# msaelices/mojo-regex

Measured on AMD Instinct MI355X. Metric: GB/s input scanned + matches/sec, 1M x 1KiB batch, [a-z]+\d+ DFA, higher is better.
Workload: dtype u8

## Files before the change

mojo_regex_amd/csrc/mrx_kernels.hip:

```cpp
#include <hip/hip_runtime.h>
#include <atomic>
#include <map>
#include <type_traits>
#include <unordered_map>
#include <chrono>

#include <cstdio>
#include <cstdlib>
#include <cstring>
#include <mutex>
#include <string>
#include <vector>

#include "../../include/mrx.h"
#include "../../include/mrx_testing.h"
#include "mrx_device.hpp"
#include "mrx_host_batch.hpp"
#include "mrx_internal.hpp"
#include "mrx_lookback.hpp"
#include "mrx_rec12.hpp"
#include "mrx_decode_bits.hpp"

using namespace mrx;

// ... 2186 lines not shown
      if (t < 0) len = 0;
      if (len > 0) addr = (uintptr_t)(data + o0);
      const int m0 = len > 0 ? (int)(addr & (CH - 1)) : 0;
      const uintptr_t rb = (addr & ~(uintptr_t)(CH - 1)) - (uintptr_t)shift;
      len_o = len; mis_o = shift + m0; flen_o = shift + m0 + len;
      *(uint4*)(tile + lane * kRowPitch + CH) =
          make_uint4((uint32_t)rb, (uint32_t)((uint64_t)rb >> 32), len > 0 ? (uint32_t)flen_o : 0u, (uint32_t)shift);
    };
    constexpr int KJ = kDynTexts / 64;
    int64_t offr[KJ + 1];
    int lenr[KJ];
#pragma unroll
    for (int j = 0; j <= KJ; ++j) {
      const int64_t t = T0 + 64 * j + lane < T1 ? T0 + 64 * j + lane : T1;
      offr[j] = vlen ? offsets[t < T1 ? t : T1 - 1] : offsets[t];
      if (j < KJ) lenr[j] = vlen ? vlen[t < T1 ? t : T1 - 1] : 0;
    }
    auto off_of = [&](int ti) -> int64_t {
      int64_t v = __shfl(offr[0], ti & 63);
#pragma unroll
      for (int j = 1; j <= KJ; ++j) { const int64_t u = __shfl(offr[j], ti & 63); v = (ti >> 6) == j ? u : v; }
      return v;
    };
    if (!vlen) {
#pragma unroll
      for (int j = 0; j < KJ; ++j) {
        const int64_t up = __shfl_down(offr[j], 1), wrap = __shfl(offr[j + 1], 0);
        lenr[j] = (int)((lane == 63 ? wrap : up) - offr[j]);
      }
    }
    auto len_of = [&](int ti) -> int {
      int v = __shfl(lenr[0], ti & 63);
#pragma unroll
      for (int j = 1; j < KJ; ++j) { const int u = __shfl(lenr[j], ti & 63); v = (ti >> 6) == j ? u : v; }
      return v;
    };
    uint16_t* perm = perm_all[wave];
    int* hist = hist_all[wave];
    {
      int mylen[KJ], tmax = 0;
#pragma unroll
      for (int j = 0; j < KJ; ++j) {
        const int ti = 64 * j + lane;
        const int l = len_of(ti < ntask ? ti : 0);
        mylen[j] = ti < ntask ? l : 0;
        tmax = max(tmax, mylen[j]);
      }
      for (int off = 32; off > 0; off >>= 1) tmax = max(tmax, __shfl_xor(tmax, off));
      const int sh = tmax >= 32 ? 32 - __builtin_clz((unsigned)tmax) - 5 : 0;
      __builtin_amdgcn_wave_barrier();
      if (lane < 32) hist[lane] = 0;
      __builtin_amdgcn_fence(__ATOMIC_RELEASE, "wavefront");
      __builtin_amdgcn_wave_barrier();
      __builtin_amdgcn_fence(__ATOMIC_ACQUIRE, "wavefront");
      int slot[KJ], cls[KJ];
#pragma unroll
      for (int j = 0; j < KJ; ++j) {
        cls[j] = 31 - (mylen[j] >> sh);
        slot[j] = 64 * j + lane < ntask ? atomicAdd(&hist[cls[j]], 1) : 0;
      }
      __builtin_amdgcn_fence(__ATOMIC_RELEASE, "wavefront");
      __builtin_amdgcn_wave_barrier();
      __builtin_amdgcn_fence(__ATOMIC_ACQUIRE, "wavefront");
      int hv = lane < 32 ? hist[lane] : 0, incl = hv;
#pragma unroll
      for (int d = 1; d < 32; d <<= 1) { const int v = __shfl_up(incl, d); if (lane >= d) incl += v; }
      __builtin_amdgcn_wave_barrier();
      if (lane < 32) hist[lane] = incl - hv;
      __builtin_amdgcn_fence(__ATOMIC_RELEASE, "wavefront");
      __builtin_amdgcn_wave_barrier();
      __builtin_amdgcn_fence(__ATOMIC_ACQUIRE, "wavefront");
#pragma unroll
      for (int j = 0; j < KJ; ++j)
        if (64 * j + lane < ntask) perm[hist[cls[j]] + slot[j]] = (uint16_t)(64 * j + lane);
      __builtin_amdgcn_fence(__ATOMIC_RELEASE, "wavefront");
      __builtin_amdgcn_wave_barrier();
      __builtin_amdgcn_fence(__ATOMIC_ACQUIRE, "wavefront");
    }
    {
      const int ti = active ? (int)perm[lane] : 0;
      const int64_t o0 = off_of(ti);
      const int l0 = len_of(ti);
      my_text = T0 + ti;
      describe(active ? my_text : -1, o0, l0, 0, my_len, mis, flen);
    }
    __builtin_amdgcn_fence(__ATOMIC_RELEASE, "wavefront");
    __builtin_amdgcn_wave_barrier();
    __builtin_amdgcn_fence(__ATOMIC_ACQUIRE, "wavefront");
    uint32_t q4 = 0;
    int start = 0, cnt = 0, wtotal = 0;
    int wrec = 0;
    bool done = false;
    int res_s = -1, res_e = -1;
    EvRec* wave_recs = MODE == ST_RECORDS ? recs + rec_region_dyn(offsets[T0], task) : nullptr;
    uint4 v[NL];
#define MRX_DYN_LOAD(CB)                                                                  \
    do {                                                                                  \
      _Pragma("unroll") for (int j_ = 0; j_ < NL; ++j_) {                                  \
        const uint4 rs_ = *(const uint4*)(tile + (RPI * j_ + rsub) * kRowPitch + CH);      \
        uint32_t fo_ = (uint32_t)(CB) + seg * 16;                                          \
        if (fo_ >= rs_.z) fo_ = rs_.w;       \
        v[j_] = MRX_LDG((const uint4*)((const uint8_t*)(((uint64_t)rs_.y << 32) | rs_.x) + fo_)); \
      }                                                                                    \
    } while (0)
    MRX_DYN_LOAD(0);
    uint8_t* wr = tile + rsub * kRowPitch + seg * 16;
    for (int cbase = 0;; cbase += CH) {
#pragma unroll
      for (int j = 0; j < NL; ++j) *(uint4*)(wr + j * RPI * kRowPitch) = v[j];
      __builtin_amdgcn_fence(__ATOMIC_RELEASE, "wavefront");
      __builtin_amdgcn_wave_barrier();
      __builtin_amdgcn_fence(__ATOMIC_ACQUIRE, "wavefront");
      const bool fin = active && (flen <= cbase + CH || (MODE == ST_SEARCH && done));
      const uint64_t fm = __ballot(fin);
      int64_t n_text = -1;
      int n_len = 0, n_mis = 0, n_flen = 0;
      if (fm) {
        const int rank = __builtin_amdgcn_mbcnt_hi((uint32_t)(fm >> 32), __builtin_amdgcn_mbcnt_lo((uint32_t)fm, 0));
        const int cpos = next + rank;
        const int cti = cpos < ntask ? (int)perm[cpos] : 0;
        const int64_t c0 = off_of(cti);
        const int cl = len_of(cti);
        if (fin) {
          n_text = cpos < ntask ? T0 + cti : -1;
          describe(n_text, c0, cl, cbase + CH, n_len, n_mis, n_flen);
        }
        next += __builtin_popcountll(fm);
        __builtin_amdgcn_fence(__ATOMIC_RELEASE, "wavefront");
        __builtin_amdgcn_wave_barrier();
        __builtin_amdgcn_fence(__ATOMIC_ACQUIRE, "wavefront");
      }
      const bool any_next = __any((active && !fin) || n_text >= 0);
      if (any_next) MRX_DYN_LOAD(cbase + CH);

      const int lim = active ? flen - cbase : 0;
      const int lo = active ? mis - cbase : 0;
      const bool all_inside = __all(lim >= CH && lo <= 0);
      uint32_t F_even = 0, meta_even = 0, sp_even = 0;
      constexpr int kUnroll = MODE == ST_COUNT ? 2 : CH / 16;
#pragma unroll kUnroll
      for (int g = 0; g < CH / 16; ++g) {
        const uint4 wv = *(const uint4*)(tile + lane * kRowPitch + g * 16);
        uint32_t words[4] = {wv.x, wv.y, wv.z, wv.w};
        if (!all_inside) {
          const int a = min(max(lo - g * 16, 0), 16), b = min(max(lim - g * 16, 0), 16);
          const uint4 pa = pmask[a], pb = pmask[b > a ? b : a];
          const uint32_t m[4] = {pb.x & ~pa.x, pb.y & ~pa.y, pb.z & ~pa.z, pb.w & ~pa.w};
#pragma unroll
          for (int j = 0; j < 4; ++j) words[j] = (words[j] & m[j]) | (fillw & ~m[j]);
        }
        uint32_t F = 0;
        if (AUTO == 4) {
          uint32_t cc[16], pi[8];
#pragma unroll
          for (int k = 0; k < 16; ++k) cc[k] = cls_lds[(words[k >> 2] >> ((k & 3) * 8)) & 0xFFu];
#pragma unroll
          for (int k = 0; k < 8; ++k) pi[k] = (cc[2 * k] << p.st_cshift) | cc[2 * k + 1];
#pragma unroll
          for (int k = 0; k < 8; ++k) {
            const uint32_t e = pair_lds[q4 + pi[k]];
            q4 = e >> 4;
            F = __builtin_amdgcn_alignbit(e, F, 4);
          }
        } else if (AUTO == 2) {
          uint32_t cc[16];
#pragma unroll
          for (int k = 0; k < 16; ++k) cc[k] = cls_lds[(words[k >> 2] >> ((k & 3) * 8)) & 0xFFu];
#pragma unroll
          for (int k = 0; k < 16; ++k) {
            const uint32_t e = tr_lds[q4 + cc[k]];
            q4 = e >> 2;
            F = __builtin_amdgcn_alignbit(e, F, 2);
          }
        } else if (AUTO == 3) {
#pragma unroll
          for (int h = 0; h < 2; ++h) {
            uint64_t cw[8];
#pragma unroll
            for (int k = 0; k < 8; ++k) cw[k] = col64_lds[(words[(8 * h + k) >> 2] >> ((k & 3) * 8)) & 0xFFu];
#pragma unroll
            for (int k = 0; k < 8; ++k) {
              const uint32_t e = (uint32_t)(cw[k] >> q4);
              q4 = e & 0x38u;
              F = __builtin_amdgcn_alignbit(e, F, 2);
            }
          }
        } else {
          uint32_t cv[16];
#pragma unroll
          for (int k = 0; k < 16; ++k) cv[k] = col_lds[(words[k >> 2] >> ((k & 3) * 8)) & 0xFFu];
#pragma unroll
          for (int k = 0; k < 16; ++k) {
            const uint32_t e = cv[k] >> q4;
            q4 = e & 0xCu;
            F = __builtin_amdgcn_alignbit(e, F, 2);
          }
        }
        const uint32_t em = F & 0xAAAAAAAAu;
        const uint32_t ns = F & 0x55555555u;
        const int gbase = cbase + g * 16 - mis;
        const uint32_t tix = (uint32_t)(my_text - T0) << kDynShift;
        if (MODE == ST_RECORDS && REC32) {
          if ((g & 1) == 0) {
            F_even = F;
            sp_even = (uint32_t)start | ((uint32_t)(gbase + kRecPosBias) << 16);
            meta_even = tix | ((uint32_t)cnt & kDynBeforeMask);
          } else {
            const bool any = ((F_even | F) & 0xAAAAAAAAu) != 0u;
            const uint64_t has = __ballot(any);
            if (has) {
              if (any) {
                const int rank = __builtin_amdgcn_mbcnt_hi((uint32_t)(has >> 32), __builtin_amdgcn_mbcnt_lo((uint32_t)has, 0));
                *(uint4*)(wave_recs + wrec + rank) = make_uint4(F_even, F, sp_even, meta_even);
              }
              wrec += __builtin_popcountll(has);
            }
          }
        } else if (MODE == ST_RECORDS) {
          const uint64_t has = __ballot(em != 0);
          if (has) {
            if (em) {
              const int rank = __builtin_amdgcn_mbcnt_hi((uint32_t)(has >> 32), __builtin_amdgcn_mbcnt_lo((uint32_t)has, 0));
              *(uint4*)(wave_recs + wrec + rank) = make_uint4(F, (uint32_t)start, (uint32_t)gbase, tix | ((uint32_t)cnt & kDynBeforeMask));
            }
            wrec += __builtin_popcountll(has);
          }
        }
        if (MODE == ST_SEARCH) {
          if (!done && em) {
            const int kk = __builtin_ctz(em) >> 1;
            const uint32_t nsb = ns & ((1u << (2 * kk)) - 1u);
            res_s = nsb ? gbase + ((31 - __builtin_clz(nsb)) >> 1) : start;
            res_e = gbase + kk;
            if (p.st_fixed_len > 0) res_s = res_e - p.st_fixed_len;
            done = true;
          }
        }
        cnt += __builtin_popcount(em);
        if (ns) start = gbase + ((31 - __builtin_clz(ns)) >> 1);
      }
      __builtin_amdgcn_wave_barrier();
      {
        const bool tail = fin && accepting(q4) && !(MODE == ST_SEARCH && done);
        if (MODE == ST_RECORDS) {
          const uint64_t has = __ballot(tail);
          if (has) {
            if (tail) {
              const int rank = __builtin_amdgcn_mbcnt_hi((uint32_t)(has >> 32), __builtin_amdgcn_mbcnt_lo((uint32_t)has, 0));
              const uint32_t meta = ((uint32_t)(my_text - T0) << kDynShift) | ((uint32_t)cnt & kDynBeforeMask);
              if (REC32) *(uint4*)(wave_recs + wrec + rank) = make_uint4(2u, 0u, (uint32_t)start | ((uint32_t)(my_len + kRecPosBias) << 16), meta);
              else *(uint4*)(wave_recs + wrec + rank) = make_uint4(2u, (uint32_t)start, (uint32_t)my_len, meta);
            }
            wrec += __builtin_popcountll(has);
          }
        }
        if (fin) {
          if (tail) ++cnt;
          if (MODE == ST_SEARCH) {
            if (!done && tail) { res_s = p.st_fixed_len > 0 ? my_len - p.st_fixed_len : start; res_e = my_len; }
            out_s[my_text] = res_s;
            out_e[my_text] = res_e;
          } else {
            counts[my_text] = cnt;
            wtotal += cnt;
          }
          my_text = n_text; active = n_text >= 0;
          my_len = n_len; mis = n_mis; flen = active ? n_flen : 0;
          q4 = 0; start = 0; cnt = 0; done = false; res_s = -1; res_e = -1;
        }
      }
      if (!any_next) break;
    }
#undef MRX_DYN_LOAD
    if (MODE == ST_RECORDS) {
      for (int off = 32; off > 0; off >>= 1) wtotal += __shfl_xor(wtotal, off);
      if (lane == 0) { wave_nrecs[task] = wrec; wave_nrecs[ntasks + task] = wtotal; }
    }
  }
}

__global__ __launch_bounds__(kBlock) void k_fused_init(unsigned long long* __restrict__ ctrl, int64_t words,
                                                       FusedArgs* __restrict__ dst, FusedArgs args) {
  for (int64_t i = (int64_t)blockIdx.x * blockDim.x + threadIdx.x; i < words; i += (int64_t)gridDim.x * blockDim.x)
    ctrl[i] = 0ull;
  if (blockIdx.x == 0 && threadIdx.x == 0) *dst = args;
}

#ifndef MRX_DECODE_TILE
#define MRX_DECODE_TILE 2048
#endif
constexpr int kDecodeTile = MRX_DECODE_TILE;
#ifndef MRX_DECODE_BATCH
#define MRX_DECODE_BATCH 8
#endif
constexpr int kDecodeBatch = MRX_DECODE_BATCH;

constexpr int kScanBlock = 256;
constexpr int kScanItems = 8;
constexpr int kScanTile = kScanBlock * kScanItems;

#ifndef MRX_DYN_DECODE_TILE
#define MRX_DYN_DECODE_TILE 2048
#endif
template <bool PACK16, bool VBASE = false, bool REC32 = false, bool DYN = false, int TILE = kDecodeTile, bool REC12 = false,
          bool LEAN = false>
__global__ __launch_bounds__(kBlock) void k_decode(int64_t n, const int32_t* __restrict__ wave_nrecs,
                                                   const EvRec* __restrict__ recs, int64_t rec_row,
                                                   const int64_t* __restrict__ offsets,
                                                   const int32_t* __restrict__ counts,
                                                   const int64_t* __restrict__ wave_base,
                                                   const int64_t* __restrict__ scan_block_sums,
                                                   int64_t* __restrict__ prefix,
                                                   int32_t* __restrict__ spans, int64_t span_cap,
                                                   int fixed_len, int64_t* __restrict__ total_out,
                                                   const int32_t* __restrict__ vbase = nullptr,
                                                   const int64_t* __restrict__ base = nullptr, int reverse = 0) {
  static_assert(!(PACK16 && VBASE), "text-relative positions of a long text do not fit 16 bits");
  static_assert(!(DYN && VBASE), "pieces are not handed out dynamically");
  static_assert(!REC12 || (REC32 && PACK16 && !VBASE && !DYN), "12-byte records: short texts at a fixed aligned pitch");
  static_assert(!LEAN || (REC32 && PACK16 && !VBASE && !DYN), "lean pass: two-word records, 16-bit positions, static tasks");
  using Slot = typename std::conditional<PACK16, uint32_t, int2>::type;
  __shared__ Slot tile_all[kBlock / 64][TILE];
  __shared__ int dense_upto[kBlock / 64][64];
  constexpr int kDecodeTile = TILE, kDecodeDirect = 3 * TILE;
  __shared__ int rel_all[DYN ? kBlock / 64 : 1][DYN ? kDynTexts : 1];
  constexpr int kTexts = DYN ? kDynTexts : 64;
  constexpr uint32_t kBefore = DYN ? kDynBeforeMask : kRecBeforeMask;
  constexpr int kTextShift = DYN ? kDynShift : 26;
  const int lane = threadIdx.x & 63;
  Slot* tile = tile_all[threadIdx.x >> 6];
  int* rel_lds = rel_all[DYN ? (threadIdx.x >> 6) : 0];
  const int64_t nw = (n + kTexts - 1) / kTexts;
  const int waves_per_block = blockDim.x >> 6;
  for (int64_t w0 = (int64_t)blockIdx.x * waves_per_block + (threadIdx.x >> 6); w0 < nw;
       w0 += (int64_t)gridDim.x * waves_per_block) {
    const int64_t w = reverse ? nw - 1 - w0 : w0;
    const int64_t first = w * kTexts;
    const int64_t i = first + lane;
    int64_t pre0 = wave_base[w] + (base ? *base : 0);
    {
      const int64_t tiles_before = w / kScanTile;
      int64_t part = 0;
      for (int64_t b = lane; b < tiles_before; b += 64) part += scan_block_sums[b];
      for (int off = 32; off > 0; off >>= 1) part += __shfl_xor(part, off);
      pre0 += part;
    }
    int my_rel = 0, total_spans = 0;
    if (DYN) {
      __builtin_amdgcn_wave_barrier();
      int carry = 0;
      for (int sb = 0; sb < kDynTexts; sb += 64) {
        const int64_t t = first + sb + lane;
        const int c = t < n ? counts[t] : 0;
        int incl = c;
#pragma unroll
        for (int d = 1; d < 64; d <<= 1) {
          const int v = __shfl_up(incl, d);
          if (lane >= d) incl += v;
        }
        rel_lds[sb + lane] = carry + incl - c;
        if (t < n) prefix[t] = pre0 + carry + incl - c;
        if (t == n - 1) { prefix[n] = pre0 + carry + incl; *total_out = pre0 + carry + incl; }
        carry += __shfl(incl, 63);
      }
      total_spans = carry;
      __builtin_amdgcn_fence(__ATOMIC_RELEASE, "wavefront");
      __builtin_amdgcn_wave_barrier();
      __builtin_amdgcn_fence(__ATOMIC_ACQUIRE, "wavefront");
    } else {
    const int my_cnt = i < n ? counts[i] : 0;
    int incl = my_cnt;
#pragma unroll
    for (int d = 1; d < 64; d <<= 1) {
      const int v = __shfl_up(incl, d);
      if (lane >= d) incl += v;
    }
    my_rel = incl - my_cnt;
    total_spans = __shfl(incl, 63);
    if (i < n) prefix[i] = pre0 + my_rel;
    if (i == n - 1) { prefix[n] = pre0 + incl; *total_out = pre0 + incl; }
    }
    const int total_recs = wave_nrecs[w];
    const EvRec* wave_recs = recs + (DYN ? rec_region_dyn(offsets[first], w)
                                         : offsets ? rec_region_start(offsets[first], w) : first * rec_row);
    const uint32_t* wave_recs12 = REC12 ? (const uint32_t*)recs + 3 * (first * rec_row) : nullptr;
    const int my_vb = (VBASE && i < n) ? vbase[i] : 0;
    if (total_spans > kDecodeDirect) {
      constexpr int kRowCap = (DYN || !PACK16) ? 0 : kDecodeTile / 64;
      int done_t = 0;
      for (int j = 0; j < total_recs; j += 64 * kDecodeBatch) {
        EvRec rr[kDecodeBatch];
#pragma unroll
        for (int u = 0; u < kDecodeBatch; ++u) {
          const int o = j + u * 64 + lane;
          rr[u].F = 0; rr[u].start = 0; rr[u].pos_base = 0; rr[u].meta = 0;
          if (o < total_recs) {
            if (REC12) {
              const uint32_t* q_ = wave_recs12 + 3 * o;
              rr[u].F = mrx_ldg32(q_); rr[u].start = (int32_t)mrx_ldg32(q_ + 1); rr[u].meta = mrx_ldg32(q_ + 2);
            } else {
            const uint4 q_ = mrx_ldg((const uint4*)(wave_recs + o));
            rr[u].F = q_.x; rr[u].start = (int32_t)q_.y; rr[u].pos_base = (int32_t)q_.z; rr[u].meta = q_.w;
            }
          }
        }
        if (kRowCap > 0) {
          dense_upto[threadIdx.x >> 6][lane] = done_t;
          __builtin_amdgcn_fence(__ATOMIC_RELEASE, "wavefront");
          __builtin_amdgcn_wave_barrier();
          __builtin_amdgcn_fence(__ATOMIC_ACQUIRE, "wavefront");
        }
#pragma unroll
        for (int u = 0; u < kDecodeBatch; ++u) {
          EvRec r = rr[u];
          const int txt = DYN ? 0 : (int)(r.meta >> 26);
          const int rel_t = DYN ? rel_lds[r.meta >> kTextShift] : __shfl(my_rel, txt);
          if (VBASE) { const int vb = __shfl(my_vb, (int)(r.meta >> 26)); r.start += vb; r.pos_base += vb; }
          const int done_r = kRowCap > 0 ? __shfl(done_t, txt) : 0;
          int within = REC12 ? rec12_before(r.meta) : (int)(r.meta & kBefore);
          int64_t dst = pre0 + rel_t + within;
          uint32_t Fw = r.F;
          int pb = REC12 ? 32 * rec12_pair(r.meta) : REC32 ? (int)((uint32_t)r.pos_base >> 16) - kRecPosBias : r.pos_base;
          int rstart = REC12 ? rec12_start(r.meta) : REC32 ? (int)((uint32_t)r.pos_base & 0xFFFFu) : r.start;
#pragma unroll
          for (int half = 0; half < (REC32 ? 2 : 1); ++half) {
            uint32_t em = Fw & 0xAAAAAAAAu;
            const uint32_t ns = Fw & 0x55555555u;
            while (em) {
              const int kk = __builtin_ctz(em) >> 1;
              const uint32_t nsb = ns & ((1u << (2 * kk)) - 1u);
              int st = nsb ? pb + ((31 - __builtin_clz(nsb)) >> 1) : rstart;
              if (fixed_len > 0) st = pb + kk - fixed_len;
              const int slot = within - done_r;
              if (kRowCap > 0 && slot < kRowCap) {
                if constexpr (PACK16) tile[txt * (kRowCap > 0 ? kRowCap : 1) + slot] = ((uint32_t)st << 16) | (uint32_t)(pb + kk);
              } else if (dst < span_cap) {
                *(int2*)(spans + 2 * dst) = make_int2(st, pb + kk);
              }
              ++dst; ++within;
              em &= em - 1;
            }
            if (REC32) {
              if (ns) rstart = pb + ((31 - __builtin_clz(ns)) >> 1);
              pb += 16;
              Fw = (uint32_t)r.start;
            }
          }
          if (kRowCap > 0 && (r.F | (REC32 ? (uint32_t)r.start : 0u)) != 0u) atomicMax(&dense_upto[threadIdx.x >> 6][txt], within);
        }
        if constexpr (PACK16 && !DYN) {
          __builtin_amdgcn_fence(__ATOMIC_RELEASE, "wavefront");
          __builtin_amdgcn_wave_barrier();
          __builtin_amdgcn_fence(__ATOMIC_ACQUIRE, "wavefront");
          const int upto_t = dense_upto[threadIdx.x >> 6][lane];
          const int64_t row_dst = pre0 + my_rel + done_t;
          int row_n = upto_t - done_t;
          if (row_n > kRowCap) row_n = kRowCap;
          for (int r_ = 0; r_ < 64; ++r_) {
            const int n_r = __shfl(row_n, r_);
            if (n_r <= 0) continue;
            const int64_t d_r = __shfl(row_dst, r_);
            if (lane < n_r && d_r + lane < span_cap) {
              const uint32_t v = (uint32_t)tile[r_ * (kRowCap > 0 ? kRowCap : 1) + lane];
              mrx_stg_span(spans + 2 * (d_r + lane), (int)(v >> 16), (int)(v & 0xFFFFu));
            }
          }
          done_t = upto_t;
          __builtin_amdgcn_wave_barrier();
        }
      }
      continue;
    }
    if constexpr (LEAN) {
      if (total_spans <= kDecodeTile) {
        const int nrec = __builtin_amdgcn_readfirstlane(total_recs), nspan = __builtin_amdgcn_readfirstlane(total_spans);
        const int last_rec = nrec - 1;
        auto lean_pass = [&](auto fixed_tag) {
          constexpr bool FIXED = decltype(fixed_tag)::value;
          for (int j = 0; j < nrec; j += 64 * kDecodeBatch) {
            uint32_t fe[kDecodeBatch], fo[kDecodeBatch], m2[kDecodeBatch], m3[kDecodeBatch];
#pragma unroll
            for (int u = 0; u < kDecodeBatch; ++u) {
              const int o = j + u * 64 + lane;
              const int oc = o < last_rec ? o : last_rec;
              if (REC12) {
                const uint32_t* q_ = wave_recs12 + 3 * oc;
                fe[u] = mrx_ldg32(q_); fo[u] = mrx_ldg32(q_ + 1); m3[u] = mrx_ldg32(q_ + 2); m2[u] = 0;
              } else {
                const uint4 q_ = mrx_ldg((const uint4*)(wave_recs + oc));
                fe[u] = q_.x; fo[u] = q_.y; m2[u] = q_.z; m3[u] = q_.w;
              }
            }
#pragma unroll
            for (int u = 0; u < kDecodeBatch; ++u) {
              if (j + u * 64 >= nrec) break;
              const bool mine = j + u * 64 + lane < nrec;
              const uint32_t f_even = mine ? fe[u] : 0u, f_odd = mine ? fo[u] : 0u;
              const uint32_t meta = m3[u];
              const int rel_t = __shfl(my_rel, (int)(meta >> 26));
              uint32_t* tp = tile + (rel_t + (REC12 ? rec12_before(meta) : (int)(meta & kBefore)));
              const int pb = REC12 ? 32 * rec12_pair(meta) : (int)(m2[u] >> 16) - kRecPosBias;
              const int rstart = REC12 ? rec12_start(meta) : (int)(m2[u] & 0xFFFFu);
              auto emit = [&](int st, int end) { *tp++ = ((uint32_t)st << 16) | (uint32_t)end; };
              decode_expand_record<FIXED>(f_even, f_odd, rstart, pb, fixed_len, emit);
            }
          }
        };
        if (fixed_len > 0) lean_pass(std::true_type{}); else lean_pass(std::false_type{});
        __builtin_amdgcn_fence(__ATOMIC_RELEASE, "wavefront");
        __builtin_amdgcn_wave_barrier();
        __builtin_amdgcn_fence(__ATOMIC_ACQUIRE, "wavefront");
        for (int k = lane; k < nspan; k += 64) {
          const int64_t dst = pre0 + k;
          if (dst < span_cap) { const uint32_t v = tile[k]; mrx_stg_span(spans + 2 * dst, (int)(v >> 16), (int)(v & 0xFFFFu)); }
        }
        __builtin_amdgcn_wave_barrier();
        continue;
      }
    }
    for (int tb = 0; tb < total_spans; tb += kDecodeTile) {
      for (int j = 0; j < total_recs; j += 64 * kDecodeBatch) {
        EvRec rr[kDecodeBatch];
#pragma unroll
        for (int u = 0; u < kDecodeBatch; ++u) {
          const int o = j + u * 64 + lane;
          rr[u].F = 0; rr[u].start = 0; rr[u].pos_base = 0; rr[u].meta = 0;
          if (o < total_recs) {
            if (REC12) {
              const uint32_t* q_ = wave_recs12 + 3 * o;
              rr[u].F = mrx_ldg32(q_); rr[u].start = (int32_t)mrx_ldg32(q_ + 1); rr[u].meta = mrx_ldg32(q_ + 2);
            } else {
            const uint4 q_ = mrx_ldg((const uint4*)(wave_recs + o));
            rr[u].F = q_.x; rr[u].start = (int32_t)q_.y; rr[u].pos_base = (int32_t)q_.z; rr[u].meta = q_.w;
            }
          }
        }
#pragma unroll
        for (int u = 0; u < kDecodeBatch; ++u) {
          EvRec r = rr[u];
          const int rel_t = DYN ? rel_lds[r.meta >> kTextShift] : __shfl(my_rel, (int)(r.meta >> 26));
          if (VBASE) { const int vb = __shfl(my_vb, (int)(r.meta >> 26)); r.start += vb; r.pos_base += vb; }
          int dst = rel_t + (REC12 ? rec12_before(r.meta) : (int)(r.meta & kBefore)) - tb;
          uint32_t Fw = r.F;
          int pb = REC12 ? 32 * rec12_pair(r.meta) : REC32 ? (int)((uint32_t)r.pos_base >> 16) - kRecPosBias : r.pos_base;
          int rstart = REC12 ? rec12_start(r.meta) : REC32 ? (int)((uint32_t)r.pos_base & 0xFFFFu) : r.start;
#pragma unroll
          for (int half = 0; half < (REC32 ? 2 : 1); ++half) {
            uint32_t em = Fw & 0xAAAAAAAAu;
            const uint32_t ns = Fw & 0x55555555u;
            while (em) {
              const int kk = __builtin_ctz(em) >> 1;
              const uint32_t nsb = ns & ((1u << (2 * kk)) - 1u);
              int st = nsb ? pb + ((31 - __builtin_clz(nsb)) >> 1) : rstart;
              if (fixed_len > 0) st = pb + kk - fixed_len;
              if (dst >= 0 && dst < kDecodeTile) {
                if constexpr (PACK16) tile[dst] = ((uint32_t)st << 16) | (uint32_t)(pb + kk);
                else tile[dst] = make_int2(st, pb + kk);
              }
              ++dst;
              em &= em - 1;
            }
            if (REC32) {
              if (ns) rstart = pb + ((31 - __builtin_clz(ns)) >> 1);
              pb += 16;
              Fw = (uint32_t)r.start;
            }
          }
        }
      }
      __builtin_amdgcn_fence(__ATOMIC_RELEASE, "wavefront");
      __builtin_amdgcn_wave_barrier();
      __builtin_amdgcn_fence(__ATOMIC_ACQUIRE, "wavefront");
      const int cnt = total_spans - tb < kDecodeTile ? total_spans - tb : kDecodeTile;
      for (int k = lane; k < cnt; k += 64) {
        const int64_t dst = pre0 + tb + k;
        if (dst < span_cap) {
          if constexpr (PACK16) { const uint32_t v = tile[k]; mrx_stg_span(spans + 2 * dst, (int)(v >> 16), (int)(v & 0xFFFFu)); }
          else { const int2 v = tile[k]; mrx_stg_span(spans + 2 * dst, v.x, v.y); }
        }
      }
      __builtin_amdgcn_wave_barrier();
    }
  }
}

constexpr int kRowsTile = 1024;
template <int G>
__global__ __launch_bounds__(kBlock) void k_decode_rows(int64_t n, const uint2* __restrict__ rows, int64_t row_pairs, int npairs,
                                                        int text_len, const int32_t* __restrict__ counts,
                                                        const int64_t* __restrict__ prefix, int32_t* __restrict__ spans,
                                                        int64_t span_cap, int fixed_len) {
  static_assert(G == 16 || G == 32 || G == 64, "lanes per text");
  constexpr int TPW = 64 / G, kTile = kRowsTile / TPW;
  __shared__ uint32_t tile_all[kBlock / 64][kRowsTile];
  const int lane = threadIdx.x & 63, gl = lane & (G - 1), grp = lane / G;
  uint32_t* tile = tile_all[threadIdx.x >> 6] + grp * kTile;
  const int64_t ngroups = (int64_t)gridDim.x * (blockDim.x >> 6) * TPW;
  auto load_pairs = [&](int64_t i, int p0) {
    const int a = p0 + 2 * gl;
    uint4 q = make_uint4(0, 0, 0, 0);
    if (i < n && a < npairs) {
      q = mrx_ldg((const uint4*)(rows + i * row_pairs + a));
      if (a + 1 >= npairs) { q.z = 0; q.w = 0; }
    }
    return q;
  };
  int64_t i = ((int64_t)blockIdx.x * (blockDim.x >> 6) + (threadIdx.x >> 6)) * TPW + grp;
  uint4 q_next = load_pairs(i, 0);
  int64_t base_next = i < n ? prefix[i] : 0;
  int total_next = i < n ? counts[i] : 0;
  for (; __any(i < n); i += ngroups) {
    uint4 q = q_next;
    const int64_t base = base_next;
    const int total_i = total_next;
    if (npairs <= 2 * G) {
      q_next = load_pairs(i + ngroups, 0);
      base_next = i + ngroups < n ? prefix[i + ngroups] : 0;
      total_next = i + ngroups < n ? counts[i + ngroups] : 0;
    }
    int carry_cnt = 0, carry_start = 0;
    for (int p0 = 0; p0 < npairs; p0 += 2 * G) {
      if (p0 > 0) q = load_pairs(i, p0);
      const uint32_t W[4] = {q.x, q.y, q.z, q.w};
      const int pb0 = 32 * (p0 + 2 * gl);
      int c = 0, ln = -1;
#pragma unroll
      for (int k = 0; k < 4; ++k) {
        c += __builtin_popcount(W[k] & 0xAAAAAAAAu);
        const uint32_t ns = W[k] & 0x55555555u;
        if (ns) ln = pb0 + 16 * k + ((31 - __builtin_clz(ns)) >> 1);
      }
      int incl = c, mx = ln;
#pragma unroll
      for (int d = 1; d < G; d <<= 1) {
        const int v = __shfl_up(incl, d, G), m = __shfl_up(mx, d, G);
        if (gl >= d) { incl += v; mx = max(mx, m); }
      }
      const int round_total = __shfl(incl, G - 1, G);
      int ex_start = __shfl_up(mx, 1, G);
      if (gl == 0) ex_start = -1;
      const int rstart0 = ex_start >= 0 ? ex_start : carry_start;
      const int before = incl - c;
      for (int tb = 0; __any(tb < round_total); tb += kTile) {
        int dst = before - tb;
        int rs = rstart0;
#pragma unroll
        for (int k = 0; k < 4; ++k) {
          uint32_t em = W[k] & 0xAAAAAAAAu;
          const uint32_t ns = W[k] & 0x55555555u;
          const int pb = pb0 + 16 * k;
          while (em) {
            const int kk = __builtin_ctz(em) >> 1;
            const uint32_t nsb = ns & ((1u << (2 * kk)) - 1u);
            int st = nsb ? pb + ((31 - __builtin_clz(nsb)) >> 1) : rs;
            if (fixed_len > 0) st = pb + kk - fixed_len;
            if (dst >= 0 && dst < kTile) tile[dst] = ((uint32_t)st << 16) | (uint32_t)(pb + kk);
            ++dst;
            em &= em - 1;
          }
          if (ns) rs = pb + ((31 - __builtin_clz(ns)) >> 1);
        }
        __builtin_amdgcn_fence(__ATOMIC_RELEASE, "wavefront");
        __builtin_amdgcn_wave_barrier();
        __builtin_amdgcn_fence(__ATOMIC_ACQUIRE, "wavefront");
        const int left = round_total - tb;
        const int cntp = left < 0 ? 0 : left < kTile ? left : kTile;
        const int64_t d0 = base + carry_cnt + tb;
        for (int k = gl; k < cntp; k += G) {
          const uint32_t v = tile[k];
          if (d0 + k < span_cap) mrx_stg_span(spans + 2 * (d0 + k), (int)(v >> 16), (int)(v & 0xFFFFu));
        }
        __builtin_amdgcn_wave_barrier();
      }
      carry_cnt += round_total;
      const int last = __shfl(mx, G - 1, G);
      if (last >= 0) carry_start = last;
    }
    if (i < n && carry_cnt < total_i && gl == 0) {
      const int64_t d = base + carry_cnt;
      if (d < span_cap) mrx_stg_span(spans + 2 * d, fixed_len > 0 ? text_len - fixed_len : carry_start, text_len);
    }
    if (npairs > 2 * G) {
      q_next = load_pairs(i + ngroups, 0);
      base_next = i + ngroups < n ? prefix[i + ngroups] : 0;
      total_next = i + ngroups < n ? counts[i + ngroups] : 0;
    }
  }
}

__global__ __launch_bounds__(kBlock) void k_first_run(DevPlan p, const uint8_t* __restrict__ blob, Layout lay, int64_t n,
                                                      int32_t* __restrict__ out_s, int32_t* __restrict__ out_e) {
  __shared__ uint8_t in_cls[256];
  for (int b = threadIdx.x; b < 256; b += blockDim.x) in_cls[b] = blob[p.off_fa_run + b];
  __syncthreads();
  const int lane = threadIdx.x & 63;
  const int64_t nwaves = (int64_t)gridDim.x * (blockDim.x >> 6);
  for (int64_t i = (int64_t)blockIdx.x * (blockDim.x >> 6) + (threadIdx.x >> 6); i < n; i += nwaves) {
    const Text t = lay.text(i);
    int run = t.len;
    if (t.len > 0) {
      const uintptr_t addr = (uintptr_t)t.ptr;
      const int mis = (int)(addr & 15);
      const uint8_t* frame = (const uint8_t*)(addr & ~(uintptr_t)15);
      const int end = mis + t.len;
      for (int blk = 0; blk < end; blk += 1024) {
        const int o = blk + 16 * lane;
        uint32_t bad = 0;
        if (o < end) {
          const uint4 v = mrx_ldg((const uint4*)(frame + o));
          const uint32_t w4[4] = {v.x, v.y, v.z, v.w};
#pragma unroll
          for (int k = 0; k < 16; ++k)
            if (!in_cls[(w4[k >> 2] >> ((k & 3) * 8)) & 0xFFu]) bad |= 1u << k;
          const int lo = mis - o, hi = end - o;
          if (lo > 0) bad &= lo >= 16 ? 0u : ~((1u << lo) - 1u);
          if (hi < 16) bad &= hi <= 0 ? 0u : ((1u << hi) - 1u);
        }
        const uint64_t any = __ballot(bad != 0u);
        if (any) {
          const int w = __builtin_ctzll(any);
          const int pos = __builtin_amdgcn_readlane(o + (bad ? __builtin_ctz(bad) : 0), w);
          run = pos - mis;
          break;
        }
      }
    }
    if (lane == 0) { out_s[i] = run > 0 ? 0 : -1; out_e[i] = run > 0 ? run : -1; }
  }
}

constexpr int kVirtBack = 256;

__device__ __forceinline__ int virt_back(const uint8_t* __restrict__ sync, const uint8_t* __restrict__ txt, int c) {
  for (int b = 1; b <= kVirtBack && b <= c; ++b)
    if (sync[txt[c - b]]) return b;
  return -1;
}
__device__ __forceinline__ int64_t virt_text_of(const int64_t* __restrict__ vfirst, int64_t n, int64_t v) {
  int64_t lo = 0, hi = n;
  while (hi - lo > 1) {
    const int64_t mid = (lo + hi) >> 1;
    if (vfirst[mid] <= v) lo = mid; else hi = mid;
  }
  return lo;
}

__global__ __launch_bounds__(kBlock) void k_virt_uniform(int64_t n, int64_t cpt, int64_t* __restrict__ vfirst) {
  for (int64_t t = (int64_t)blockIdx.x * blockDim.x + threadIdx.x; t <= n; t += (int64_t)gridDim.x * blockDim.x)
    vfirst[t] = t * cpt;
}
__global__ __launch_bounds__(kBlock) void k_virt_count(Layout lay, int64_t n, int C, int32_t* __restrict__ cnt) {
  for (int64_t t = (int64_t)blockIdx.x * blockDim.x + threadIdx.x; t < n; t += (int64_t)gridDim.x * blockDim.x) {
    const int len = lay.text(t).len;
    cnt[t] = len <= C ? 1 : (len + C - 1) / C;
  }
}

__global__ __launch_bounds__(kBlock) void k_virt_check(Layout lay, int64_t n, const int64_t* __restrict__ vfirst,
                                                       int64_t nv, int C, const uint8_t* __restrict__ sync,
                                                       int32_t* __restrict__ back) {
  for (int64_t v = (int64_t)blockIdx.x * blockDim.x + threadIdx.x; v < nv; v += (int64_t)gridDim.x * blockDim.x) {
    const int64_t t = virt_text_of(vfirst, n, v);
    const int k = (int)(v - vfirst[t]);
    back[v] = k == 0 ? 0 : virt_back(sync, lay.text(t).ptr, k * C);
  }
}

__global__ __launch_bounds__(kBlock) void k_virt_fill(Layout lay, int64_t n, const int64_t* __restrict__ vfirst,
                                                      int64_t nv, int C, const int32_t* __restrict__ back,
                                                      int64_t* __restrict__ vstart, int32_t* __restrict__ vlen,
                                                      uint32_t* __restrict__ vskip, int32_t* __restrict__ vbase,
                                                      int disjoint) {
  for (int64_t v = (int64_t)blockIdx.x * blockDim.x + threadIdx.x; v < nv; v += (int64_t)gridDim.x * blockDim.x) {
    const int64_t t = virt_text_of(vfirst, n, v);
    const int64_t v0 = vfirst[t];
    const int k = (int)(v - v0), cpt = (int)(vfirst[t + 1] - v0);
    const Text tx = lay.text(t);
    const int64_t abs0 = tx.ptr - lay.data;
    const int b = back[v];
    const int64_t c = (int64_t)k * C;
    int64_t st = abs0 + c;
    int ln = 0, base = (int)c;
    uint32_t sk = 0;
    if (b >= 0) {
      int j = k + 1;
      while (j < cpt && back[v0 + j] == -1) ++j;
      const int e = j == cpt ? tx.len : (disjoint ? j * C - back[v0 + j] : j * C);
      st = abs0 + c - b; ln = e - (int)c + b; base = (int)c - b;
      sk = disjoint ? 0u : ((uint32_t)b | (e == tx.len ? 0x80000000u : 0u));
    }
    vstart[v] = st; vlen[v] = ln; vskip[v] = sk; vbase[v] = base;
  }
}

__global__ __launch_bounds__(kBlock) void k_candidate_density(DevPlan p, const uint8_t* __restrict__ blob,
                                                              const uint8_t* __restrict__ data, int64_t nbytes,
                                                              unsigned int* __restrict__ hits) {
  __shared__ uint8_t starts[256];
  const uint8_t* cls = blob + p.off_cls;
  const uint8_t* first = blob + p.off_first;
  const uint16_t* tr = (const uint16_t*)(blob + p.off_trans);
  const bool filt = (p.flags & PF_HAS_MATCHER) != 0;
  for (int b = threadIdx.x; b < 256; b += blockDim.x) starts[b] = (tr[cls[b]] != 0xFFFFu && (!filt || first[b])) ? 1 : 0;
  __syncthreads();
  unsigned int k = 0;
  for (int64_t i = (int64_t)blockIdx.x * blockDim.x + threadIdx.x; i < nbytes; i += (int64_t)gridDim.x * blockDim.x) k += starts[data[i]];
  for (int off = 32; off > 0; off >>= 1) k += __shfl_xor(k, off);
  if ((threadIdx.x & 63) == 0 && k) atomicAdd(hits, k);
}
__global__ __launch_bounds__(kBlock) void k_virt_add_base(int64_t nv, const int64_t* __restrict__ vprefix,
                                                          const int32_t* __restrict__ vbase, int32_t* __restrict__ spans,
                                                          int64_t span_cap) {
  __shared__ int64_t range[2];
  const int64_t total = vprefix[nv] < span_cap ? vprefix[nv] : span_cap;
  constexpr int kPer = 4;
  for (int64_t k0 = (int64_t)blockIdx.x * kBlock * kPer; k0 < total; k0 += (int64_t)gridDim.x * kBlock * kPer) {
    const int64_t k1 = k0 + kBlock * kPer - 1 < total - 1 ? k0 + kBlock * kPer - 1 : total - 1;
    __syncthreads();
    if (threadIdx.x < 128) {
      const int lane = threadIdx.x & 63;
      const int64_t k = threadIdx.x < 64 ? k0 : k1;
// ... 4342 lines not shown
```

Measured before the change: 3448.

## Prefetch first decode record batch before prefix scan in lean decode path

Hoists the first batch of record loads in the lean decode path so it is issued before the wave's prefix computation (the block-sum reduction and count scan). The record fetch latency can then overlap that scalar/scan work. The block-sum reduction is also restructured: the first 64 entries are loaded directly, the remainder is unrolled four at a time, and the 64-bit wave sum uses split 16/16/32-bit group scans. Several wave-uniform values are made scalar via readfirstlane, and the lean branch now runs before the direct-decode branch. In exchange, register pressure rises because the record batch stays live across the scan, and it relies on empty asm to keep the loads early.

```diff
diff --git a/mojo_regex_amd/csrc/mrx_kernels.hip b/mojo_regex_amd/csrc/mrx_kernels.hip
--- a/mojo_regex_amd/csrc/mrx_kernels.hip
+++ b/mojo_regex_amd/csrc/mrx_kernels.hip
@@ -2512,6 +2512,17 @@
 #ifndef MRX_DYN_DECODE_TILE
 #define MRX_DYN_DECODE_TILE 2048
 #endif
+template <int G, bool XOR>
+__device__ __forceinline__ int group_scan(int x);
+
+__device__ __forceinline__ int64_t wave_sum64(int64_t v) {
+  const uint32_t lo = (uint32_t)v, hi = (uint32_t)((uint64_t)v >> 32);
+  const uint32_t s0 = (uint32_t)__builtin_amdgcn_readlane(group_scan<64, false>((int)(lo & 0xFFFFu)), 63);
+  const uint32_t s1 = (uint32_t)__builtin_amdgcn_readlane(group_scan<64, false>((int)(lo >> 16)), 63);
+  const uint32_t s2 = (uint32_t)__builtin_amdgcn_readlane(group_scan<64, false>((int)hi), 63);
+  return (int64_t)((uint64_t)s0 + ((uint64_t)s1 << 16) + ((uint64_t)s2 << 32));
+}
+
 template <bool PACK16, bool VBASE = false, bool REC32 = false, bool DYN = false, int TILE = kDecodeTile, bool REC12 = false,
           bool LEAN = false>
 __global__ __launch_bounds__(kBlock) void k_decode(int64_t n, const int32_t* __restrict__ wave_nrecs,
@@ -2542,19 +2553,62 @@
   int* rel_lds = rel_all[DYN ? (threadIdx.x >> 6) : 0];
   const int64_t nw = (n + kTexts - 1) / kTexts;
   const int waves_per_block = blockDim.x >> 6;
-  for (int64_t w0 = (int64_t)blockIdx.x * waves_per_block + (threadIdx.x >> 6); w0 < nw;
+  const int wave_in_block = __builtin_amdgcn_readfirstlane((int)(threadIdx.x >> 6));
+  for (int64_t w0 = (int64_t)blockIdx.x * waves_per_block + wave_in_block; w0 < nw;
        w0 += (int64_t)gridDim.x * waves_per_block) {
     const int64_t w = reverse ? nw - 1 - w0 : w0;
     const int64_t first = w * kTexts;
     const int64_t i = first + lane;
-    int64_t pre0 = wave_base[w] + (base ? *base : 0);
-    {
-      const int64_t tiles_before = w / kScanTile;
-      int64_t part = 0;
-      for (int64_t b = lane; b < tiles_before; b += 64) part += scan_block_sums[b];
-      for (int off = 32; off > 0; off >>= 1) part += __shfl_xor(part, off);
-      pre0 += part;
-    }
+    const int64_t tiles_before = w / kScanTile;
+    const int64_t wbase = wave_base[w];
+    const int total_recs = __builtin_amdgcn_readfirstlane(wave_nrecs[w]);
+    const int64_t base0 = base ? *base : 0;
+    const EvRec* wave_recs = recs + (DYN ? rec_region_dyn(offsets[first], w)
+                                         : offsets ? rec_region_start(offsets[first], w) : first * rec_row);
+    const uint32_t* wave_recs12 = REC12 ? (const uint32_t*)recs + 3 * (first * rec_row) : nullptr;
+    const int my_cnt = (!DYN && i < n) ? counts[i] : 0;
+    int64_t part = lane < tiles_before ? scan_block_sums[lane] : 0;
+    uint32_t fe[kDecodeBatch], fo[kDecodeBatch], m2[kDecodeBatch], m3[kDecodeBatch];
+    const int last_rec = total_recs - 1;
+    auto load_batch = [&](int j) {
+#pragma unroll
+      for (int u = 0; u < kDecodeBatch; ++u) {
+        const int o = j + u * 64 + lane;
+        const int oc = o < last_rec ? o : last_rec;
+        if (REC12) {
+          const uint32_t* q_ = wave_recs12 + 3 * oc;
+          fe[u] = mrx_ldg32(q_); fo[u] = mrx_ldg32(q_ + 1); m3[u] = mrx_ldg32(q_ + 2); m2[u] = 0;
+        } else {
+          const uint4 q_ = mrx_ldg((const uint4*)(wave_recs + oc));
+          fe[u] = q_.x; fo[u] = q_.y; m2[u] = q_.z; m3[u] = q_.w;
+        }
+      }
+    };
+    auto retire_batch = [&]() {
+#pragma unroll
+      for (int u = 0; u < kDecodeBatch; ++u) {
+        asm volatile("" ::"v"(fe[u]), "v"(fo[u]), "v"(m3[u]));
+        if (!REC12) asm volatile("" ::"v"(m2[u]));
+      }
+    };
+    if constexpr (LEAN) {
+      if (total_recs > 0) {
+        load_batch(0);
+      } else {
+#pragma unroll
+        for (int u = 0; u < kDecodeBatch; ++u) fe[u] = fo[u] = m2[u] = m3[u] = 0;
+      }
+    }
+    if (tiles_before > 64) {
+      for (int64_t b = 64 + lane; b < tiles_before; b += 256) {
+        const int64_t p0 = scan_block_sums[b];
+        const int64_t p1 = b + 64 < tiles_before ? scan_block_sums[b + 64] : 0;
+        const int64_t p2 = b + 128 < tiles_before ? scan_block_sums[b + 128] : 0;
+        const int64_t p3 = b + 192 < tiles_before ? scan_block_sums[b + 192] : 0;
+        part += (p0 + p1) + (p2 + p3);
+      }
+    }
+    const int64_t pre0 = wbase + base0 + wave_sum64(part);
     int my_rel = 0, total_spans = 0;
     if (DYN) {
       __builtin_amdgcn_wave_barrier();
@@ -2573,28 +2627,54 @@
         if (t == n - 1) { prefix[n] = pre0 + carry + incl; *total_out = pre0 + carry + incl; }
         carry += __shfl(incl, 63);
       }
-      total_spans = carry;
+      total_spans = __builtin_amdgcn_readfirstlane(carry);
       __builtin_amdgcn_fence(__ATOMIC_RELEASE, "wavefront");
       __builtin_amdgcn_wave_barrier();
       __builtin_amdgcn_fence(__ATOMIC_ACQUIRE, "wavefront");
     } else {
-    const int my_cnt = i < n ? counts[i] : 0;
-    int incl = my_cnt;
-#pragma unroll
-    for (int d = 1; d < 64; d <<= 1) {
-      const int v = __shfl_up(incl, d);
-      if (lane >= d) incl += v;
-    }
+    const int incl = group_scan<64, false>(my_cnt);
     my_rel = incl - my_cnt;
-    total_spans = __shfl(incl, 63);
+    total_spans = __builtin_amdgcn_readlane(incl, 63);
+    if constexpr (LEAN) retire_batch();
     if (i < n) prefix[i] = pre0 + my_rel;
     if (i == n - 1) { prefix[n] = pre0 + incl; *total_out = pre0 + incl; }
     }
-    const int total_recs = wave_nrecs[w];
-    const EvRec* wave_recs = recs + (DYN ? rec_region_dyn(offsets[first], w)
-                                         : offsets ? rec_region_start(offsets[first], w) : first * rec_row);
-    const uint32_t* wave_recs12 = REC12 ? (const uint32_t*)recs + 3 * (first * rec_row) : nullptr;
     const int my_vb = (VBASE && i < n) ? vbase[i] : 0;
+    if constexpr (LEAN) {
+      if (total_spans <= kDecodeTile) {
+        const int nrec = total_recs, nspan = total_spans;
+        auto lean_pass = [&](auto fixed_tag) {
+          constexpr bool FIXED = decltype(fixed_tag)::value;
+          for (int j = 0; j < nrec; j += 64 * kDecodeBatch) {
+            if (j > 0) load_batch(j);
+#pragma unroll
+            for (int u = 0; u < kDecodeBatch; ++u) {
+              if (j + u * 64 >= nrec) break;
+              const bool mine = j + u * 64 + lane < nrec;
+              const uint32_t f_even = mine ? fe[u] : 0u, f_odd = mine ? fo[u] : 0u;
+              const uint32_t meta = m3[u];
+              const int rel_t = __shfl(my_rel, (int)(meta >> 26));
+              uint32_t* tp = tile + (rel_t + (REC12 ? rec12_before(meta) : (int)(meta & kBefore)));
+              const int pb = REC12 ? 32 * rec12_pair(meta) : (int)(m2[u] >> 16) - kRecPosBias;
+              const int rstart = REC12 ? rec12_start(meta) : (int)(m2[u] & 0xFFFFu);
+              auto emit = [&](int st, int end) { *tp++ = ((uint32_t)st << 16) | (uint32_t)end; };
+              decode_expand_record<FIXED>(f_even, f_odd, rstart, pb, fixed_len, emit);
+            }
+          }
+        };
+        if (fixed_len > 0) lean_pass(std::true_type{}); else lean_pass(std::false_type{});
+        retire_batch();
+        __builtin_amdgcn_fence(__ATOMIC_RELEASE, "wavefront");
+        __builtin_amdgcn_wave_barrier();
+        __builtin_amdgcn_fence(__ATOMIC_ACQUIRE, "wavefront");
+        for (int k = lane; k < nspan; k += 64) {
+          const int64_t dst = pre0 + k;
+          if (dst < span_cap) { const uint32_t v = tile[k]; mrx_stg_span(spans + 2 * dst, (int)(v >> 16), (int)(v & 0xFFFFu)); }
+        }
+        __builtin_amdgcn_wave_barrier();
+        continue;
+      }
+    }
     if (total_spans > kDecodeDirect) {
       constexpr int kRowCap = (DYN || !PACK16) ? 0 : kDecodeTile / 64;
       int done_t = 0;
@@ -2680,53 +2760,6 @@
         }
       }
       continue;
-    }
-    if constexpr (LEAN) {
-      if (total_spans <= kDecodeTile) {
-        const int nrec = __builtin_amdgcn_readfirstlane(total_recs), nspan = __builtin_amdgcn_readfirstlane(total_spans);
-        const int last_rec = nrec - 1;
-        auto lean_pass = [&](auto fixed_tag) {
-          constexpr bool FIXED = decltype(fixed_tag)::value;
-          for (int j = 0; j < nrec; j += 64 * kDecodeBatch) {
-            uint32_t fe[kDecodeBatch], fo[kDecodeBatch], m2[kDecodeBatch], m3[kDecodeBatch];
-#pragma unroll
-            for (int u = 0; u < kDecodeBatch; ++u) {
-              const int o = j + u * 64 + lane;
-              const int oc = o < last_rec ? o : last_rec;
-              if (REC12) {
-                const uint32_t* q_ = wave_recs12 + 3 * oc;
-                fe[u] = mrx_ldg32(q_); fo[u] = mrx_ldg32(q_ + 1); m3[u] = mrx_ldg32(q_ + 2); m2[u] = 0;
-              } else {
-                const uint4 q_ = mrx_ldg((const uint4*)(wave_recs + oc));
-                fe[u] = q_.x; fo[u] = q_.y; m2[u] = q_.z; m3[u] = q_.w;
-              }
-            }
-#pragma unroll
-            for (int u = 0; u < kDecodeBatch; ++u) {
-              if (j + u * 64 >= nrec) break;
-              const bool mine = j + u * 64 + lane < nrec;
-              const uint32_t f_even = mine ? fe[u] : 0u, f_odd = mine ? fo[u] : 0u;
-              const uint32_t meta = m3[u];
-              const int rel_t = __shfl(my_rel, (int)(meta >> 26));
-              uint32_t* tp = tile + (rel_t + (REC12 ? rec12_before(meta) : (int)(meta & kBefore)));
-              const int pb = REC12 ? 32 * rec12_pair(meta) : (int)(m2[u] >> 16) - kRecPosBias;
-              const int rstart = REC12 ? rec12_start(meta) : (int)(m2[u] & 0xFFFFu);
-              auto emit = [&](int st, int end) { *tp++ = ((uint32_t)st << 16) | (uint32_t)end; };
-              decode_expand_record<FIXED>(f_even, f_odd, rstart, pb, fixed_len, emit);
-            }
-          }
-        };
-        if (fixed_len > 0) lean_pass(std::true_type{}); else lean_pass(std::false_type{});
-        __builtin_amdgcn_fence(__ATOMIC_RELEASE, "wavefront");
-        __builtin_amdgcn_wave_barrier();
-        __builtin_amdgcn_fence(__ATOMIC_ACQUIRE, "wavefront");
-        for (int k = lane; k < nspan; k += 64) {
-          const int64_t dst = pre0 + k;
-          if (dst < span_cap) { const uint32_t v = tile[k]; mrx_stg_span(spans + 2 * dst, (int)(v >> 16), (int)(v & 0xFFFFu)); }
-        }
-        __builtin_amdgcn_wave_barrier();
-        continue;
-      }
     }
     for (int tb = 0; tb < total_spans; tb += kDecodeTile) {
       for (int j = 0; j < total_recs; j += 64 * kDecodeBatch) {
```

Result: faster. 3525 (median of 6 runs) (+2.2%).
